# neuromodulation/py_neuromodulation

Measured on AMD Instinct MI355X. Metric: windows/sec (all features), 256 ch @ 1 kHz, higher is better.
Workload: dtype f32; 1 GPU; 256ch/GPU @1kHz, W=1000, hop=100, 1024 hops/step, all 9 hot-path features, 4 bands, notch50+CAR, z-score normalisation; channels_per_gpu=256, features_per_window=9984, parallelism=channel-shard x1, no collective

## Files before the change

### py_neuromodulation_amd/csrc/nmx_engine.inc

```

#include <algorithm>
#include <chrono>
#include <cmath>
#include <cstdio>
#include <cstdlib>
#include <cstring>
#include <map>
#include <string>
#include <thread>
#include <deque>
#include <functional>
#include <mutex>
#include <condition_variable>
#include <pthread.h>
#include <vector>

#include "../../include/nmx.h"
#include "nmx_k_coh.h"
#include "nmx_k_proj.h"

static thread_local std::string g_nmx_err;
static int nmx_fail(int code, const std::string& msg) {
  g_nmx_err = msg;
  return code;
// ... 88 lines not shown
  bool have_sharp = false;
  NmxCohArgs coh{};
  bool have_coh = false;
  float* d_R = nullptr;
  bool car = false;
  float car_diag = 0.f, car_off = 0.f;
  bool rs_ok = false;
  NmxRerefStructArgs rst{};
  int nt_timeosc = 64, nt_bank = 256, nt_thr = 256;
  int chunk_windows = 1024;
  bool sharp_dense_first = false;
  bool thr_wave = true;
  bool thr_fill = true;
  bool fill_split = true;
  bool thr_list_lds = true;
  bool tiny_inline = true;
  bool starts_mod4 = false;
  long long burst_windows_seen = 0;
  Buf thr_slots;
  Buf to_todo;
  Buf rn_qt, rn_qn;
  Buf tap;
  Buf x_in, x_in2[2], x_ref, x_rs, x_rn, rn_mean, rn_scale, x_pf[2], y_notch, yb, out, starts, mask;
  Buf win_pin;
  Buf env[2], swy[2], thr[2], sw_todo[2];
  Buf sw_slab;
  float* d_top = nullptr;
  long long* d_counts = nullptr;
  size_t top_bytes = 0, counts_bytes = 0;
  NmxKalmanArgs kal{};
  bool have_kalman = false;
  NmxResampleArgs rs{};
  bool have_resample = false;
  NmxRawNormArgs rn{};
  bool have_rawnorm = false;
  bool rn_sorted_valid = false;
  long long rn_hops = 0;
  size_t rn_ring_bytes = 0, rn_cnt_bytes = 0, rn_len_bytes = 0;
  std::vector<std::vector<double>> pre_taps;
  int w_in = 0;
  int nt_resample = 256;
  double* d_kf = nullptr;
  size_t kf_bytes = 0;
  be_timer_t timers[9];
// ... 62 lines not shown
```

### py_neuromodulation_amd/csrc/nmx_engine_abi.inc

```

extern "C" {

int nmx_abi_version(void) { return NMX_ABI_VERSION; }
int nmx_device_count(void) { return be_device_count(); }
const char* nmx_last_error(void) { return g_nmx_err.c_str(); }

int nmx_plan_destroy(nmx_plan* plan) {
  Plan* P = (Plan*)plan;
  if (!P) return 0;
  be_set_device(P->device);
  be_sync(P->stream);
  be_sync(P->stream_b);
  be_sync(P->stream_d);
  be_sync(P->stream_f);
  for (void* t : P->tables) be_free(t);
  for (Buf* b : {&P->tap, &P->rn_qt, &P->rn_qn, &P->thr_slots, &P->to_todo, &P->x_dc, &P->x_in, &P->x_ref, &P->x_rs, &P->x_rn, &P->rn_mean, &P->rn_scale, &P->x_pf[0], &P->x_pf[1], &P->sw_todo[0], &P->sw_todo[1], &P->sw_slab, &P->y_notch, &P->env[0], &P->env[1], &P->swy[0], &P->swy[1], &P->yb, &P->thr[0], &P->thr[1], &P->out, &P->starts, &P->mask})
    if (b->p) be_free(b->p);
  if (P->d_top) be_free(P->d_top);
  if (P->d_counts) be_free(P->d_counts);
  if (P->d_R) be_free(P->d_R);
  if (P->d_dc_sub) be_free(P->d_dc_sub);
  if (P->d_dc_pref) be_free(P->d_dc_pref);
  if (P->d_dc_nanv) be_free(P->d_dc_nanv);
  if (P->d_kf) be_free(P->d_kf);
  if (P->rn.ring) be_free(P->rn.ring);
  if (P->rn.count) be_free(P->rn.count);
  if (P->rn.len) be_free(P->rn.len);
  if (P->win_pin.p) be_host_free(P->win_pin.p);
  for (auto& t : P->timers) be_timer_destroy(t);
  be_event_destroy(P->ev_fork);
  be_event_destroy(P->ev_join[0]);
  be_event_destroy(P->ev_join[1]);
  be_event_destroy(P->ev_main[0]);
  be_event_destroy(P->ev_main[1]);
// ... 211 lines not shown
int nmx_state_reset(nmx_plan* plan) {
  Plan* P = (Plan*)plan;
  if (!P) return nmx_fail(NMX_E_INVALID, "null plan");
  dc_reset(*P);
  if (!P->have_bursts && !P->have_kalman && !P->have_rawnorm) return 0;
  be_set_device(P->device);
  be_sync(P->stream);
  if (P->last_stream && P->last_stream != P->stream) be_sync(P->last_stream);
  be_sync(P->stream_b);
  be_sync(P->stream_d);
  be_sync(P->stream_f);
  if (P->have_rawnorm) rawnorm_reset(*P);
  if (P->have_bursts) {
    be_memset_sync(P->d_top, 0, P->top_bytes);
    be_memset_sync(P->d_counts, 0, P->counts_bytes);
    P->burst_windows_seen = 0;
  }
  if (P->have_kalman) kalman_reset(*P);
  return 0;
}

int nmx_state_size(const nmx_plan* plan, int64_t* n_bytes) {
  const Plan* P = (const Plan*)plan;
  if (!P || !n_bytes) return nmx_fail(NMX_E_INVALID, "null argument");
  *n_bytes = (int64_t)(P->top_bytes + P->counts_bytes + P->kf_bytes + dc_state_bytes(*P) + rn_state_bytes(*P));
  return 0;
}

int nmx_state_export(nmx_plan* plan, void* dst, int64_t n_bytes) {
  Plan* P = (Plan*)plan;
// ... 31 lines not shown
  if (P->have_rawnorm && (size_t)n_bytes >= fixed + 2 * sizeof(long long))
    memcpy(&src_cap, (const char*)src + fixed + sizeof(long long), sizeof(long long));
  NMX_REQUIRE(!P->have_rawnorm || (src_cap > 0 && src_cap < (1ll << 31)), "state blob: bad raw-normaliser header");
  NMX_REQUIRE((size_t)n_bytes == fixed + (P->have_rawnorm ? rn_state_bytes_cap(*P, src_cap) : 0), "state size mismatch");
  if (!n_bytes) return 0;
  dc_state_import(*P, (const char*)src + P->top_bytes + P->counts_bytes + P->kf_bytes);
  be_set_device(P->device);
  be_sync(P->stream);
  if (P->last_stream && P->last_stream != P->stream) be_sync(P->last_stream);
  be_sync(P->stream_b);
  be_sync(P->stream_f);
  if (P->have_bursts) {
    be_h2d_sync(P->d_top, src, P->top_bytes);
    be_h2d_sync(P->d_counts, (const char*)src + P->top_bytes, P->counts_bytes);
    memcpy(&P->burst_windows_seen, (const char*)src + P->top_bytes + sizeof(long long), sizeof(long long));
  }
  if (P->have_kalman) be_h2d_sync(P->d_kf, (const char*)src + P->top_bytes + P->counts_bytes, P->kf_bytes);
  if (P->have_rawnorm) {
    const char* q = (const char*)src + P->top_bytes + P->counts_bytes + P->kf_bytes;
    memcpy(&P->rn_hops, q, sizeof(long long)); q += 2 * sizeof(long long);
    const int C = P->d.n_channels, cap = P->rn.cap;
    const float* ring_src = (const float*)q;
    const char* cnt_src = q + (size_t)C * (size_t)src_cap * sizeof(float);
    const char* len_src = cnt_src + P->rn_cnt_bytes;
    if (src_cap == cap) {
      be_h2d_sync(P->rn.ring, ring_src, P->rn_ring_bytes);
    } else {
      std::vector<float> ring((size_t)C * cap, 0.f);
      for (int c = 0; c < C; ++c) {
        long long cnt;
// ... 16 lines not shown
```

### py_neuromodulation_amd/csrc/nmx_engine_plan_state.inc

```
static void rawnorm_reset(Plan& P) {
  be_memset_sync(P.rn.ring, 0, P.rn_ring_bytes);
  be_memset_sync(P.rn.count, 0, P.rn_cnt_bytes);
  be_memset_sync(P.rn.len, 0, P.rn_len_bytes);
  P.rn_hops = 0;
  P.rn_sorted_valid = false;
}

int build_rawnorm(Plan& P) {
  const nmx_plan_desc& d = P.d;
  if (d.raw_norm_method <= 0) return 0;
  NMX_REQUIRE(d.raw_norm_method >= NMX_RAWNORM_MEAN && d.raw_norm_method <= NMX_RAWNORM_POWER,
              "raw normalisation method outside 1..8 (mean, zscore, median, zscore-median, robust, minmax, quantile, power)");
  NMX_REQUIRE(d.raw_norm_n >= 2 && d.raw_norm_add >= 1 && d.raw_norm_add <= d.window,
              "raw normalisation: need N >= 2 and 1 <= int(sfreq / feat_hz) <= window");
  NmxRawNormArgs& A = P.rn;
  A.n_channels = d.n_channels; A.W = d.window;
  A.add = d.raw_norm_add; A.keep = d.raw_norm_n - 1;
  A.cap = std::max(d.window, A.keep) + A.add + 64;
  A.method = d.raw_norm_method; A.clip = d.raw_norm_clip;
  P.rn_ring_bytes = (size_t)d.n_channels * A.cap * sizeof(float);
  P.rn_cnt_bytes = (size_t)d.n_channels * sizeof(long long);
  P.rn_len_bytes = (size_t)d.n_channels * sizeof(int);
  A.ring = (float*)be_alloc(P.rn_ring_bytes);
  A.count = (long long*)be_alloc(P.rn_cnt_bytes);
// ... 66 lines not shown
    A.pad_mode = 0;
    A.n_sw_filters = 1;
    const int L = d.n_pre_taps[i];
    NMX_REQUIRE(L & 1, "pre-filter taps must have odd length");
    const int half = (L - 1) / 2, uh = std::min(half, A.W - 1);
    NmxFilterDev& F = A.f[0];
    F.half = uh;
    F.bp_seglen = 0;
    F.burst_index = -1;
    F.sw_index = 0;
    F.store_raw = 0;
    int rc = build_fir_stage(P, {P.pre_taps[i].data() + (half - uh)}, FirRules{uh, 1024, false, false, 1}, &P.pre[i]);
    if (rc) return rc;
  }
  return 0;
}

int build_bursts(Plan& P) {
  const nmx_plan_desc& d = P.d;
  if (!(d.features & NMX_F_BURSTS)) return 0;
  NMX_REQUIRE(d.n_burst_bands > 0, "bursts enabled without burst bands");
  int nb = 0;
  for (int i = 0; i < d.n_filters; ++i) nb += d.filters[i].burst_index >= 0;
  NMX_REQUIRE(nb == d.n_burst_bands, "every burst band needs exactly one filter");
  NmxBurstThrArgs& T = P.bthr;
  T.n_channels = d.n_channels;
  T.n_bands = d.n_burst_bands;
  T.W = d.window;
  T.q = d.burst_threshold / 100.0;
  NMX_REQUIRE(T.q >= 0.0 && T.q <= 1.0, "burst threshold must be a percentile in [0, 100]");
// ... 28 lines not shown
  S.n_channels = d.n_channels;
  S.n_bands = d.n_burst_bands;
  S.W = d.window;
  S.sfreq = (float)d.sfreq;
  S.seg_s = (float)seg_s;
  S.out_mask = d.burst_out_mask;
  S.cols = cv(d.burst_cols);
  S.off_e = 0;
  S.off_red = al4(d.window + d.window / 16 + 1);
  S.lds_floats = S.off_red + 64;
  const size_t n_state = (size_t)d.n_channels * d.n_burst_bands;
  P.top_bytes = n_state * T.K * sizeof(float);
  P.counts_bytes = n_state * 2 * sizeof(long long);
  P.d_top = (float*)be_alloc(P.top_bytes);
  P.d_counts = (long long*)be_alloc(P.counts_bytes);
  if (!P.d_top || !P.d_counts) return nmx_fail(NMX_E_NOMEM, "burst state allocation failed");
  be_memset_sync(P.d_top, 0, P.top_bytes);
  be_memset_sync(P.d_counts, 0, P.counts_bytes);
  P.have_bursts = true;
  return 0;
}

int build_resample(Plan& P) {
  const nmx_plan_desc& d = P.d;
  if (d.raw_window <= 0) return 0;
  NMX_REQUIRE(d.resample_ratio > 0 && d.resample_ratio != 1.0, "resample_ratio must be positive and != 1");
  NMX_REQUIRE(d.raw_window >= 4 && d.raw_window <= 65336, "raw_window must be in [4, 65 336] samples");
  const double ratio = d.resample_ratio;
  const int W = d.raw_window;
  const int final_len = (int)std::nearbyint(ratio * W);
  NMX_REQUIRE(final_len == d.window, "window must equal round(resample_ratio * raw_window)");
  const int min_add = std::min(W / 8, 100) * 2;
  int n_pad = 1;
// ... 260 lines not shown
```

### py_neuromodulation_amd/csrc/nmx_engine_run.inc

```
static int run_prep_stages(Plan& P, const float*& src, long long& ch_stride, long long& win_stride,
                           const long long*& starts, int nw, int& clean, be_stream_t s, const NmxBankArgs* fuse_bank = nullptr) {
  const int C = P.d.n_channels, W = P.d.window, Wi = P.w_in;
  int rc;
  auto take = [&](const void* y, int w) {
    src = (const float*)y;
    ch_stride = w; win_stride = (long long)C * w; starts = nullptr; clean = 0;
  };
  for (size_t i = 0; i < P.pre.size(); ++i) {
    Buf& dst = P.x_pf[i & 1];
    if ((rc = ensure(dst, (size_t)nw * C * Wi * sizeof(float)))) return rc;
    NmxBankArgs A = P.pre[i].a;
    A.x = src; A.ch_stride = ch_stride; A.win_stride = win_stride; A.starts = starts; A.clean_on_load = clean;
    A.out = nullptr; A.sw_out = (float*)dst.p;
    launch_fir_stage(P, P.pre[i], A, nw * C, s);
    take(dst.p, Wi);
  }
  if (P.have_notch) {
    if ((rc = ensure(P.y_notch, (size_t)nw * C * Wi * sizeof(float)))) return rc;
    NmxBankArgs A = P.notch.a;
    A.x = src; A.ch_stride = ch_stride; A.win_stride = win_stride; A.starts = starts; A.clean_on_load = clean;
    A.out = nullptr; A.y_out = (float*)P.y_notch.p;
#ifndef NMX_HOST_EMU
    if (fuse_bank) launch_notch_bank_fused(P, A, *fuse_bank, nw * C, s);
    else
// ... 19 lines not shown
static int run_chunk(Plan& P, const float* d_x, long long ldx, long long lo, long long hi,
                     const long long* d_starts, int nw, float* d_out, be_stream_t s, bool timed,
                     float* d_pre = nullptr, const int64_t* h_starts = nullptr) {
  const long long n_range = hi - lo;
  const nmx_plan_desc& d = P.d;
  const int C = d.n_channels, W = d.window;
  int rc;
  const int par = (int)(P.chunk_seq & 1);
  if (P.chunk_seq >= 2) {
    be_stream_wait(s, P.ev_join[par]);
    be_stream_wait(s, P.ev_join_d[par]);
  }
  if (P.overlap == 1 && P.chunk_seq >= 1)
    be_stream_wait(s, P.ev_join[par ^ 1]);
  Buf& B_env = P.env[par];
  Buf& B_swy = P.swy[par];
  Buf& B_thr = P.thr[par];
  Buf& B_todo = P.sw_todo[par];
  const float* src = d_x;
  long long ch_stride = ldx, win_stride = 0;
  const long long* starts = d_starts;
  int clean = 1;
  bool raw_live = true;
  const bool tev = timed && nw >= 8;
  if (timed) be_stage_reset();
  if (tev) be_timer_start(P.timers[1], s);
  be_stage(1);
  if (P.d_R) {
    if ((rc = ensure(P.x_ref, (size_t)C * n_range * sizeof(float)))) return rc;
    launch_reref(P, d_x + lo, ldx, (float*)P.x_ref.p, n_range, n_range, s);
// ... 111 lines not shown
    be_event_record(P.ev_fork_d, s);
    be_stream_wait(P.stream_d, P.ev_fork_d);
    if ((rc = launch_sharp(P.stream_d))) return rc;
    be_event_record(P.ev_join_d[par], P.stream_d);
  }
  be_stream_t sb = s;
  be_stage(4);
  if (P.have_bursts) {
    if ((rc = ensure(B_thr, (size_t)nw * C * d.n_burst_bands * sizeof(float)))) return rc;
    if (P.overlap == 1) {
      sb = P.stream_b;
      be_event_record(P.ev_fork, s);
      be_stream_wait(sb, P.ev_fork);
    }
    if (tev) be_timer_start(P.timers[4], sb);
    if (P.bank.w64 || P.bank.a.partitioned) {
      NmxHilbertArgs H = P.hil;
      H.y = (const float*)P.yb.p; H.env = (float*)B_env.p;
      be_launch_hilbert(H, P.hil_kind, (long long)nw * C * d.n_burst_bands, (size_t)H.lds_floats * 4, sb);
    }
    if (P.overlap >= 2) {
      sb = P.stream_b;
      be_event_record(P.ev_fork, s);
      be_stream_wait(sb, P.ev_fork);
    }
    NmxBurstThrArgs T = P.bthr;
    T.env = (const float*)B_env.p; T.thr = (float*)B_thr.p; T.top = P.d_top; T.counts = P.d_counts;
    T.n_windows = nw;
    const int n_seq = C * d.n_burst_bands;
    auto hops = [&](int first, int n) {
      NmxBurstThrArgs X = T;
      X.env = T.env + (size_t)first * n_seq * W;
      X.thr = T.thr + (size_t)first * n_seq;
      X.n_windows = n;
      return X;
    };
    int done = 0;
    if (P.thr_fill && P.burst_windows_seen == 0 && nw >= 2) {
      int n = nmx_burst_fill_hops(T, nw);
#ifndef NMX_HOST_EMU
      if (P.thr_wave)
        for (int k = 1; k < n; ++k)
// ... 17 lines not shown
        for (int k = 1; k < rem; ++k)
          if (nmx_burst_thr_wave_ok(T, seen + k)) { k_fill = k; break; }
      }
#endif
      if (k_fill > 0 && k_fill < rem) {
        be_launch_burst_thr(hops(done, k_fill), n_seq, P.nt_thr, (size_t)T.lds_floats * 4, sb, -1, P.thr_list_lds);
        be_launch_burst_thr(hops(done + k_fill, rem - k_fill), n_seq, P.nt_thr, (size_t)T.lds_floats * 4, sb, seen + k_fill,
                            P.thr_list_lds);
      } else {
        be_launch_burst_thr(hops(done, rem), n_seq, P.nt_thr, (size_t)T.lds_floats * 4, sb, P.thr_wave ? seen : -1, P.thr_list_lds);
      }
    }
    P.burst_windows_seen += nw;
    NmxBurstStatArgs S = P.bstat;
    S.env = (const float*)B_env.p; S.thr = (const float*)B_thr.p; S.out = d_out; S.n_windows = nw;
    be_launch_burst_stat(S, nw * C * d.n_burst_bands, (size_t)S.lds_floats * 4, sb);
    if (tev) be_timer_stop(P.timers[4], sb);
    if (P.overlap) be_event_record(P.ev_join[par], sb);
  }
  if (P.have_to) {
    NmxTimeOscArgs A = P.to;
    A.x = src; A.ch_stride = ch_stride; A.win_stride = win_stride; A.starts = starts;
    A.out = d_out; A.clean_on_load = clean;
    A.starts_mod4 = (!starts || P.starts_mod4) ? 1 : 0;
    A.dcf = dcf;
    if (dcf && !P.to_takes_dc) {
      if ((rc = with_dc())) return rc;
      A.x = src_dc; A.ch_stride = W; A.win_stride = (long long)C * W; A.starts = nullptr; A.clean_on_load = 0; A.dcf = nullptr;
    }
    A.todo = nullptr;
// ... 462 lines not shown
    be_launch_rs64_elem(A, NMX_RS64_MUL, nullptr, cur, L, C, s);
    fft(cur, oth, ld, L, +1, C);
  }
  be_launch_rs64_elem(A, NMX_RS64_OUT, cur, nullptr, final_len, C, s);
  be_d2h_2d_async(y, (size_t)ldy * sizeof(double), d + nx, (size_t)final_len * sizeof(double), (size_t)final_len * sizeof(double),
                  (size_t)C, s);
  rc = be_sync(s);
  be_stream_destroy(s);
  be_free(d);
  return rc ? rc : be_check_launch();
}

int nmx_last_kernels(nmx_plan* plan, int which, char* buf, int64_t n) {
  Plan* P = (Plan*)plan;
  if (!P || !buf || n < 1 || which < 1 || which > 8) return nmx_fail(NMX_E_INVALID, "bad argument");
  const std::string& k = P->kernels[which];
  const size_t m = std::min<size_t>(k.size(), (size_t)n - 1);
  memcpy(buf, k.data(), m);
  buf[m] = 0;
  return 0;
}
```

### py_neuromodulation_amd/csrc/nmx_k_bank_w64.h

```cpp
#pragma once

#include "nmx_k_bank.h"
#include "nmx_k_fft500.h"
#include "nmx_k_sharpwave.h"

#ifdef NMX_HOST_EMU
#define NMX_UNROLL
#else
#define NMX_UNROLL _Pragma("unroll")
#endif

#ifdef NMX_HOST_EMU
#define NMX_SCHED_FENCE() ((void)0)
#else
#define NMX_SCHED_FENCE() __builtin_amdgcn_sched_barrier(0)
#endif

#if defined(NMX_BANK_PROFILE) && !defined(NMX_HOST_EMU)
#define NMX_PROF_DECL long long pf_t = clock64(), pf_acc[8] = {0, 0, 0, 0, 0, 0, 0, 0};
#define NMX_PROF(i) { const long long t_ = clock64(); pf_acc[i] += t_ - pf_t; pf_t = t_; }
#define NMX_PROF_PRINT(w, c)                                                                                          \
  if ((w) == 5 && ((c) == 3 || (c) == 40) && (threadIdx.x & 63) == 0)                                                  \
    printf("bank profile w=%d c=%d: load+fwd %lld | spectral+passA %lld | passB load+dft %lld | passB store %lld | "  \
           "passC %lld | variance %lld | series stores %lld | partners %lld (cycles, whole item, %d filters)\n", (w), (c), pf_acc[0],   \
// ... 643 lines not shown
    NMX_PROF(7)
  }
  NMX_PROF_PRINT(w, c)
}

struct NmxHilbertArgs {
  const float* y;
  float* env;
  int W;
  NmxFft hil_r;
  NmxFft hil_c;
  int hil_full;
  int off_a, off_b, off_y, lds_floats;
  const float* w500_tab;
  const float* w1000_tab;
};

NMX_DEV void nmx_hilbert_item(const NmxHilbertArgs& A, long long item, float* smem) {
  float2* bufA = (float2*)(smem + A.off_a);
  float2* bufB = (float2*)(smem + A.off_b);
  const int W = A.W, Wh = W >> 1;
  const float* src = A.y + item * W;
  float* dst = A.env + item * W;
  if (!A.hil_full) {
    float* ys = smem + A.off_y;
    float* pk = (float*)bufB;
    nmx_stage_row(src, W, [=](int i, float v) { pk[i] = v; ys[i] = v; });
    NMX_SYNC();
    const float2* Zy = nmx_fft_auto<-1, true>(A.hil_r, bufB, bufA, bufB);
    float2* Yb = (Zy == bufA) ? bufB : bufA;
// ... 22 lines not shown
  const float invW = 1.f / (float)W;
  for (int k = NMX_TID; k < W; k += NMX_NT) {
    float2 val = make_float2(0.f, 0.f);
    if (k == 0) val = Zy[0];
    else if (k <= (W - 1) / 2) val = make_float2(2.f * Zy[k].x, 2.f * Zy[k].y);
    Ab[k] = make_float2(val.x * invW, val.y * invW);
  }
  NMX_SYNC();
  float2* Zbuf = (Ab == bufA) ? bufB : bufA;
  const float2* an = nmx_fft_auto<+1, true>(A.hil_c, Ab, Zbuf, Ab);
  for (int i = NMX_TID; i < W; i += NMX_NT) dst[i] = nmx_sqrt_fast(an[i].x * an[i].x + an[i].y * an[i].y);
}

#ifndef NMX_HOST_EMU
#define NMX_W500_LDS_FLOATS (1008 + 1000)
NMX_DEV void nmx_hilbert_w500_item(const NmxHilbertArgs& A, long long item, float* smem) {
  const int l = NMX_TID;
  nmx_c2* hb = (nmx_c2*)smem;
  nmx_c2* ha = hb + 504;
#ifdef NMX_DEBUG_HILBERT_SAMEROW
  const nmx_rsrc rin = nmx_make_rsrc(A.y + (item & 1023) * 1000, 4000);
#else
  const nmx_rsrc rin = nmx_make_rsrc(A.y + item * 1000, 4000);
#endif
  const nmx_rsrc rout = nmx_make_rsrc(A.env + item * 1000, 4000);
  NmxW500TwReg T;
  T.load(A.w500_tab, l);
  nmx_c2 y[8];
#pragma unroll
  for (int q = 0; q < 8; ++q) y[q] = __builtin_amdgcn_raw_buffer_load_b64(rin, 8 * l + 512 * q, 0, 0);
#pragma unroll
  for (int q = 0; q < 8; ++q)
    if (q < 7 || l < 52) hb[l + 64 * q] = y[q];
  NMX_WAVE_FENCE();
  const nmx_c2* ht = nmx_w500_hilbert(ha, hb, T, (const nmx_c2*)A.w500_tab + NMX_W500_TW_N, l);
#pragma unroll
  for (int q = 0; q < 8; ++q) {
    const nmx_c2 h = ht[l + 64 * q];
    const nmx_c2 e = nmx_mk2(nmx_sqrt_fast(y[q].x * y[q].x + h.x * h.x), nmx_sqrt_fast(y[q].y * y[q].y + h.y * h.y));
    __builtin_amdgcn_raw_buffer_store_b64(e, rout, 8 * l + 512 * q, 0, 0);
  }
}
#define NMX_W1000_LDS_FLOATS 2000
NMX_DEV void nmx_hilbert_w1000_item(const NmxHilbertArgs& A, long long item, float* smem) {
  const int l = NMX_TID;
  nmx_c2* hb = (nmx_c2*)smem;
  nmx_c2* ha = hb;
  const nmx_rsrc rin = nmx_make_rsrc(A.y + item * 2000, 8000);
  const nmx_rsrc rout = nmx_make_rsrc(A.env + item * 2000, 8000);
  NmxW1000TwReg T;
  T.load(A.w1000_tab, l);
  nmx_c2 y[16];
#pragma unroll
  for (int q = 0; q < 16; ++q) y[q] = __builtin_amdgcn_raw_buffer_load_b64(rin, 8 * l + 512 * q, 0, 0);
#pragma unroll
  for (int q = 0; q < 16; ++q)
    if (q < 15 || l < 40) hb[l + 64 * q] = y[q];
  NMX_WAVE_FENCE();
  const nmx_c2* ht = nmx_w1000_hilbert(ha, hb, T, (const nmx_c2*)A.w1000_tab + NMX_W1000_TW_N, l);
#pragma unroll
  for (int q = 0; q < 16; ++q) {
    if (!(q < 15 || l < 40)) continue;
    const nmx_c2 h = ht[l + 64 * q];
    const nmx_c2 e = nmx_mk2(nmx_sqrt_fast(y[q].x * y[q].x + h.x * h.x), nmx_sqrt_fast(y[q].y * y[q].y + h.y * h.y));
    __builtin_amdgcn_raw_buffer_store_b64(e, rout, 8 * l + 512 * q, 0, 0);
  }
}
#endif
```

### py_neuromodulation_amd/csrc/nmx_k_burst_stat_reg.h

```cpp
#pragma once

#include "nmx_k_bank_w64.h"
#include "nmx_k_bursts.h"

#ifndef NMX_HOST_EMU
template <int CH>
NMX_DEV void nmx_burst_stat_item_reg(const NmxBurstStatArgs& A, int w, int c, int bi) {
  const int l = NMX_TID, W = A.W;
  const long long item = ((long long)w * A.n_channels + c) * A.n_bands + bi;
  const nmx_rsrc rs = nmx_make_rsrc(A.env + item * W, 4 * W);
  float v[CH];
#pragma unroll
  for (int q = 0; q < CH / 4; ++q) {
    typedef unsigned u4 __attribute__((ext_vector_type(4)));
    const u4 t = __builtin_amdgcn_raw_buffer_load_b128(rs, 4 * (l * CH + 4 * q), 0, 0);
    v[4 * q] = __uint_as_float(t.x); v[4 * q + 1] = __uint_as_float(t.y);
    v[4 * q + 2] = __uint_as_float(t.z); v[4 * q + 3] = __uint_as_float(t.w);
  }
  const float thr = A.thr[item];
  const int i0 = l * CH;
  const int n = W - i0 < 0 ? 0 : (W - i0 > CH ? CH : W - i0);
  float tail = 0.f;
  int zpos = -1;
#pragma unroll
// ... 70 lines not shown
```

### py_neuromodulation_amd/csrc/nmx_k_bursts.h

```cpp
#pragma once

#include "nmx_device.h"
#ifdef NMX_HOST_EMU
#include <cstdio>
#include <cstdlib>
#include <vector>
#endif

struct NmxBurstThrArgs {
  const float* env;
  float* thr;
  float* top;
  long long* counts;
  int n_windows, n_channels, n_bands, W;
  int K;
  int n_ring;
  int overlap;
  double q;
  int P2;
  int off_l0, off_l1, off_p, off_red, lds_floats;
  int list_in_global;
};

NMX_DEV void nmx_bitonic_desc(float* p, int n2) {
  for (int k = 2; k <= n2; k <<= 1) {
    for (int j = k >> 1; j > 0; j >>= 1) {
      for (int i = NMX_TID; i < n2; i += NMX_NT) {
        const int ixj = i ^ j;
        if (ixj > i) {
          const float a = p[i], b = p[ixj];
          const bool desc = ((i & k) == 0);
          if (desc ? (a < b) : (a > b)) {
            p[i] = b;
            p[ixj] = a;
          }
        }
      }
// ... 242 lines not shown
      Lm = nmx_merge_into<CH>(L, Lm, K, ps, ins, nP, vals);
      for (int j = NMX_TID; j < nF; j += NMX_NT) L[Lm + j] = F[nF - 1 - j];
      NMX_SYNC();
      nF = NMX_THR_FREFILL;
      Lm = K - nF;
      nP = 0;
      for (int j = NMX_TID; j < nF; j += NMX_NT) F[j] = L[K - 1 - j];
      NMX_SYNC();
    }
  }
  NMX_SYNC();
  if (!A.list_in_global) for (int i = NMX_TID; i < len; i += NMX_NT) gtop[i] = L[i];
  if (NMX_TID == 0) {
    A.counts[2 * sidx] = total;
    A.counts[2 * sidx + 1] = nwin;
  }
}

#ifndef NMX_HOST_EMU
#define NMX_THRW_PF 16
#define NMX_THRW_I 256
#define NMX_THRW_PF_LL 8
#define NMX_THRW_PF_OF(NR, LL) ((NR) == 2 ? ((LL) ? NMX_THRW_PF_LL : NMX_THRW_PF) : 4)
#define NMX_THRW_LDS_FLOATS_OF(NR, LL) (2 * 256 * (NR) + 3 * ((NR) == 2 ? NMX_THR_P : 512) + NMX_THRW_I + NMX_THRW_PF_OF(NR, LL) * 64 * (NR))
#define NMX_THRW_LDS_FLOATS_NR(NR) NMX_THRW_LDS_FLOATS_OF(NR, false)
#define NMX_THRW_LDS_FLOATS NMX_THRW_LDS_FLOATS_NR(2)

NMX_DEV int nmx_count_ge_lds(const float* l, int n, float v) {
  int lo = 0, hi = n;
  while (lo < hi) {
// ... 360 lines not shown
      }
    }
  }
#ifdef NMX_THRW_PROFILE
  if (lane == 0 && (sidx == 0 || sidx == 311))
    printf("[thrw %lld] hops %d inserts %d flushes %d | cycles: top %lld classify %lld fringe %lld store %lld sort %lld stream %lld recut %lld\n",
           sidx, A.n_windows, n_ins, n_flush, tp[0], tp[1], tp[2], tp[3], tp[4], tp[5], tp[6]);
#endif
  if (LL) {
    NMX_WAVE_FENCE();
    for (int j = lane; j < K; j += 64) Lg[j] = L[j];
  }
  if (lane == 0) {
    A.counts[2 * sidx] = total;
    A.counts[2 * sidx + 1] = nwin;
  }
}
#endif

struct NmxBurstStatArgs {
  const float* env;
  const float* thr;
  float* out;
  int n_outputs, n_windows, n_channels, n_bands, W;
  float sfreq, seg_s;
  unsigned out_mask;
  NmxCols cols;
  int off_e, off_red, lds_floats;
};

#ifdef NMX_HOST_EMU
NMX_DEV double nmx_wave_excl_sum_d(double v, double* total) { *total = v; return 0.0; }
NMX_DEV void nmx_wave_excl_latest(int& pos, double& val) { pos = -1; val = 0.0; }
#else
NMX_DEV double nmx_dpp_d(double v, double ident, int ctrl_sel) {
  const long long vb = __builtin_bit_cast(long long, v), ib = __builtin_bit_cast(long long, ident);
  int lo = (int)(vb & 0xffffffffll), hi = (int)(vb >> 32);
  const int ilo = (int)(ib & 0xffffffffll), ihi = (int)(ib >> 32);
  switch (ctrl_sel) {
    case 0: lo = __builtin_amdgcn_update_dpp(ilo, lo, 0x111, 0xf, 0xf, false); hi = __builtin_amdgcn_update_dpp(ihi, hi, 0x111, 0xf, 0xf, false); break;
    case 1: lo = __builtin_amdgcn_update_dpp(ilo, lo, 0x112, 0xf, 0xf, false); hi = __builtin_amdgcn_update_dpp(ihi, hi, 0x112, 0xf, 0xf, false); break;
    case 2: lo = __builtin_amdgcn_update_dpp(ilo, lo, 0x114, 0xf, 0xf, false); hi = __builtin_amdgcn_update_dpp(ihi, hi, 0x114, 0xf, 0xf, false); break;
    case 3: lo = __builtin_amdgcn_update_dpp(ilo, lo, 0x118, 0xf, 0xf, false); hi = __builtin_amdgcn_update_dpp(ihi, hi, 0x118, 0xf, 0xf, false); break;
    case 4: lo = __builtin_amdgcn_update_dpp(ilo, lo, 0x142, 0xa, 0xf, false); hi = __builtin_amdgcn_update_dpp(ihi, hi, 0x142, 0xa, 0xf, false); break;
// ... 31 lines not shown
    const double tv = nmx_dpp_d(v, 0.0, st);
    if (tp > p) { p = tp; v = tv; }
  }
  pos = nmx_dpp_i(p, -1, 6);
  val = nmx_dpp_d(v, 0.0, 6);
}
#endif

#define NMX_EP(i) ((i) + ((i) >> 4))

NMX_DEV void nmx_burst_stat_item(const NmxBurstStatArgs& A, int w, int c, int bi, float* smem) {
  float* e = smem + A.off_e;
  float* red = smem + A.off_red;
  const int W = A.W;
  const long long item = ((long long)w * A.n_channels + c) * A.n_bands + bi;
  const float* src = A.env + item * W;
  nmx_stage_row(src, W, [=](int i, float v) { e[NMX_EP(i)] = v; });
  NMX_SYNC();
  const float thr = A.thr[item];
  const int chunk = (W + NMX_NT - 1) / NMX_NT;
  const int i0 = NMX_TID * chunk, i1 = (i0 + chunk) < W ? (i0 + chunk) : W;
  double csum = 0.0;
  int zpos = -1;
  double zpre = 0.0;
  for (int i = i0; i < i1; ++i) {
    const float ev = e[NMX_EP(i)];
    csum += (double)ev;
    if (!(ev >= thr)) { zpos = i; zpre = csum; }
  }
  double total;
// ... 61 lines not shown
```

### py_neuromodulation_amd/csrc/nmx_wave.hip

```cpp
#ifndef NMX_NT_FIXED
#error "compile with -DNMX_NT_FIXED=64"
#endif
#include <hip/hip_runtime.h>
#include <cstdio>
#include <cstdlib>

#include <cstdlib>

#include "nmx_k_bursts.h"
#include "nmx_k_bank_w64.h"
#include "nmx_k_burst_stat_reg.h"
#include "nmx_k_scan.h"
#include "nmx_k_td.h"
#include "nmx_k_timeosc_w1000.h"
#include "nmx_k_timeosc_w510.h"
#include "nmx_k_sharpwave.h"

extern __shared__ __attribute__((aligned(16))) float nmx_smem_wave[];

static int waves_per_wg(size_t lds_one, int dflt = 1) {
  const char* v = getenv("NMX_WAVES_PER_WG");
  const int k = (v && atoi(v) >= 1 && atoi(v) <= 4) ? atoi(v) : 0;
  int kk = k ? k : dflt;
  while (kk > 1 && lds_one * kk > 64 * 1024) --kk;
// ... 1 lines not shown
}
#define NMX_WAVE_ITEM(item, smem, n_items, slice)                                                   \
  const int wave_ = __builtin_amdgcn_readfirstlane((int)(threadIdx.x >> 6));                        \
  const int item = (int)blockIdx.x * (int)(blockDim.x >> 6) + wave_;                                \
  if (item >= (n_items)) return;                                                                    \
  float* smem = nmx_smem_wave + wave_ * (slice)

__global__ void __launch_bounds__(256) nmx_kern_burst_stat(const NmxBurstStatArgs A, int n_items, int slice) {
  const int wave = __builtin_amdgcn_readfirstlane((int)(threadIdx.x >> 6));
  const int item = blockIdx.x * (blockDim.x >> 6) + wave;
  if (item >= n_items) return;
  const int bi = item % A.n_bands, r = item / A.n_bands;
  nmx_burst_stat_item(A, r / A.n_channels, r % A.n_channels, bi, nmx_smem_wave + wave * slice);
}

template <int CH>
__global__ void __launch_bounds__(256) nmx_kern_burst_stat_reg(const NmxBurstStatArgs A, int n_items) {
  const int wave = __builtin_amdgcn_readfirstlane((int)(threadIdx.x >> 6));
  const int item = blockIdx.x * 4 + wave;
  if (item >= n_items) return;
  const int bi = item % A.n_bands, r = item / A.n_bands;
  nmx_burst_stat_item_reg<CH>(A, r / A.n_channels, r % A.n_channels, bi);
}

__global__ void __launch_bounds__(256) nmx_kern_sharp(const NmxSharpArgs A, int n_items, int slice) {
  const int wave = __builtin_amdgcn_readfirstlane((int)(threadIdx.x >> 6));
  const int item = blockIdx.x * (blockDim.x >> 6) + wave;
  if (item >= n_items) return;
  const int fi = item % A.n_filters, r = item / A.n_filters;
  nmx_sharp_item(A, r / A.n_channels, r % A.n_channels, fi, nmx_smem_wave + wave * slice);
}

template <int NR, bool LL>
__global__ void __launch_bounds__(64) nmx_kern_burst_thr_wave(const NmxBurstThrArgs A) {
  __builtin_amdgcn_s_setprio(3);
  const int item = blockIdx.x;
  nmx_burst_thr_wave_item<NR, LL>(A, item / A.n_bands, item % A.n_bands, nmx_smem_wave);
// ... 12 lines not shown
  const long long per_round = 256LL * (long long)((160 * 1024) / with_list);
  const bool ll = lds_list && nr == 2 && with_list <= 80 * 1024 && windows_seen < 4096 && (long long)n_items <= 2 * per_round;
  const size_t lds = ll ? with_list : base;
  if (nr == 2) {
    if (ll) hipLaunchKernelGGL((nmx_kern_burst_thr_wave<2, true>), dim3(n_items), dim3(64), lds, s, *A);
    else hipLaunchKernelGGL((nmx_kern_burst_thr_wave<2, false>), dim3(n_items), dim3(64), lds, s, *A);
    nmxi_note_kernel(ll ? "nmx_kern_burst_thr_wave<2, true>" : "nmx_kern_burst_thr_wave<2, false>");
  } else {
    hipLaunchKernelGGL((nmx_kern_burst_thr_wave<4, false>), dim3(n_items), dim3(64), lds, s, *A);
    nmxi_note_kernel("nmx_kern_burst_thr_wave<4, false>");
  }
}

__global__ void __launch_bounds__(256) nmx_kern_hilbert_w500(const NmxHilbertArgs A, int n_items) {
  NMX_WAVE_ITEM(item, smem, n_items, NMX_W500_LDS_FLOATS);
  nmx_hilbert_w500_item(A, (long long)item, smem);
}

extern "C" void nmx_wave_launch_hilbert_w500(const NmxHilbertArgs* A, long long n_items, hipStream_t s) {
  const int k = waves_per_wg((size_t)NMX_W500_LDS_FLOATS * 4);
  hipLaunchKernelGGL(nmx_kern_hilbert_w500, dim3((unsigned)((n_items + k - 1) / k)), dim3(64 * k),
                     (size_t)NMX_W500_LDS_FLOATS * 4 * k, s, *A, (int)n_items);
  nmxi_note_kernel("nmx_kern_hilbert_w500");
}

__global__ void __launch_bounds__(256) nmx_kern_hilbert_w1000(const NmxHilbertArgs A, long long n_items) {
  const int wave = __builtin_amdgcn_readfirstlane((int)(threadIdx.x >> 6));
  const long long item = (long long)blockIdx.x * 4 + wave;
  if (item >= n_items) return;
  nmx_hilbert_w1000_item(A, item, nmx_smem_wave + wave * NMX_W1000_LDS_FLOATS);
}

extern "C" void nmx_wave_launch_hilbert_w1000(const NmxHilbertArgs* A, long long n_items, hipStream_t s) {
  static unsigned long long seen = 0;
  if (nmx_first_on_device(seen))
    (void)hipFuncSetAttribute((const void*)nmx_kern_hilbert_w1000, hipFuncAttributeMaxDynamicSharedMemorySize, 160 * 1024);
  hipLaunchKernelGGL(nmx_kern_hilbert_w1000, dim3((unsigned)((n_items + 3) / 4)), dim3(256), (size_t)4 * NMX_W1000_LDS_FLOATS * 4, s, *A, n_items);
  nmxi_note_kernel("nmx_kern_hilbert_w1000");
}

template <int NB, unsigned SPEC = 0>
__global__ void __launch_bounds__(256) nmx_kern_timeosc_w1000(const NmxTimeOscArgs A, int n_items, int slice) {
  NMX_WAVE_ITEM(item, smem, n_items, slice);
  const int w = nmx_uniform_i(item / A.n_channels), c = nmx_uniform_i(item % A.n_channels);
  NmxW500TwReg T;
  T.load(A.w500_tab, (int)(threadIdx.x & 63));
  NmxTdRegs R;
  nmx_td_load<1000>(A, w, c, R);
  nmx_timeosc_w1000_body<NB, false, NmxW500TwReg, false, SPEC>(A, w, c, R, T, smem);
}

// ... 224 lines not shown
    (void)hipFuncSetAttribute((const void*)nmx_kern_sharp_todo, hipFuncAttributeMaxDynamicSharedMemorySize, 160 * 1024);
  }
  const int blocks = (n_items + 63) / 64;
  const int grid = blocks < 256 * 14 ? blocks : 256 * 14;
  hipLaunchKernelGGL(nmx_kern_sharp_todo, dim3(grid), dim3(64), lds, s, *A, n_items, todo);
  nmxi_note_kernel("nmx_kern_sharp_todo");
}

extern "C" void nmx_wave_launch_burst_stat(const NmxBurstStatArgs* A, int n_items, size_t lds, hipStream_t s) {
  static unsigned long long seen = 0;
  if (nmx_first_on_device(seen)) {
    (void)hipFuncSetAttribute((const void*)nmx_kern_burst_stat, hipFuncAttributeMaxDynamicSharedMemorySize, 160 * 1024);
  }
  if ((A->W & 3) == 0 && A->W <= 2048) {
    if (A->W <= 1024) {
      hipLaunchKernelGGL(nmx_kern_burst_stat_reg<16>, dim3((n_items + 3) / 4), dim3(256), 0, s, *A, n_items);
      nmxi_note_kernel("nmx_kern_burst_stat_reg<16>");
    } else {
      hipLaunchKernelGGL(nmx_kern_burst_stat_reg<32>, dim3((n_items + 3) / 4), dim3(256), 0, s, *A, n_items);
      nmxi_note_kernel("nmx_kern_burst_stat_reg<32>");
    }
    return;
  }
  const int k = waves_per_wg(lds);
  const int slice = (int)((lds / 4 + 3) & ~(size_t)3);
  hipLaunchKernelGGL(nmx_kern_burst_stat, dim3((n_items + k - 1) / k), dim3(64 * k), (size_t)slice * 4 * k, s, *A,
                     n_items, slice);
  nmxi_note_kernel("nmx_kern_burst_stat");
}

extern "C" void nmx_wave_launch_sharp(const NmxSharpArgs* A, int n_items, size_t lds, hipStream_t s) {
  if (A->slab_mode) { nmx_wave_launch_sharp_slab(A, n_items, nullptr, s); return; }
  static unsigned long long seen = 0;
  if (nmx_first_on_device(seen)) {
    (void)hipFuncSetAttribute((const void*)nmx_kern_sharp, hipFuncAttributeMaxDynamicSharedMemorySize, 160 * 1024);
// ... 8 lines not shown
```

Measured before the change: 152,400 windows/s.

## Skip envelope stores and burst stats for rows below running burst threshold floor

```diff
diff --git a/py_neuromodulation_amd/csrc/nmx_engine.inc b/py_neuromodulation_amd/csrc/nmx_engine.inc
--- a/py_neuromodulation_amd/csrc/nmx_engine.inc
+++ b/py_neuromodulation_amd/csrc/nmx_engine.inc
@@ -126,6 +126,9 @@
   bool thr_fill = true;
   bool fill_split = true;
   bool thr_list_lds = true;
+  bool env_sparse = true;
+  bool env_sparse_count = false;
+  long long env_tail_rows = 0, env_rows = 0;
   bool tiny_inline = true;
   bool starts_mod4 = false;
   long long burst_windows_seen = 0;
@@ -136,10 +139,12 @@
   Buf x_in, x_in2[2], x_ref, x_rs, x_rn, rn_mean, rn_scale, x_pf[2], y_notch, yb, out, starts, mask;
   Buf win_pin;
   Buf env[2], swy[2], thr[2], sw_todo[2];
+  Buf env_full[2];
   Buf sw_slab;
   float* d_top = nullptr;
   long long* d_counts = nullptr;
   size_t top_bytes = 0, counts_bytes = 0;
+  float* d_floor = nullptr;
   NmxKalmanArgs kal{};
   bool have_kalman = false;
   NmxResampleArgs rs{};
diff --git a/py_neuromodulation_amd/csrc/nmx_engine_abi.inc b/py_neuromodulation_amd/csrc/nmx_engine_abi.inc
--- a/py_neuromodulation_amd/csrc/nmx_engine_abi.inc
+++ b/py_neuromodulation_amd/csrc/nmx_engine_abi.inc
@@ -14,10 +14,11 @@
   be_sync(P->stream_d);
   be_sync(P->stream_f);
   for (void* t : P->tables) be_free(t);
-  for (Buf* b : {&P->tap, &P->rn_qt, &P->rn_qn, &P->thr_slots, &P->to_todo, &P->x_dc, &P->x_in, &P->x_ref, &P->x_rs, &P->x_rn, &P->rn_mean, &P->rn_scale, &P->x_pf[0], &P->x_pf[1], &P->sw_todo[0], &P->sw_todo[1], &P->sw_slab, &P->y_notch, &P->env[0], &P->env[1], &P->swy[0], &P->swy[1], &P->yb, &P->thr[0], &P->thr[1], &P->out, &P->starts, &P->mask})
+  for (Buf* b : {&P->tap, &P->rn_qt, &P->rn_qn, &P->thr_slots, &P->to_todo, &P->x_dc, &P->x_in, &P->x_ref, &P->x_rs, &P->x_rn, &P->rn_mean, &P->rn_scale, &P->x_pf[0], &P->x_pf[1], &P->sw_todo[0], &P->sw_todo[1], &P->sw_slab, &P->y_notch, &P->env[0], &P->env[1], &P->env_full[0], &P->env_full[1], &P->swy[0], &P->swy[1], &P->yb, &P->thr[0], &P->thr[1], &P->out, &P->starts, &P->mask})
     if (b->p) be_free(b->p);
   if (P->d_top) be_free(P->d_top);
   if (P->d_counts) be_free(P->d_counts);
+  if (P->d_floor) be_free(P->d_floor);
   if (P->d_R) be_free(P->d_R);
   if (P->d_dc_sub) be_free(P->d_dc_sub);
   if (P->d_dc_pref) be_free(P->d_dc_pref);
@@ -259,6 +260,7 @@
   if (P->have_bursts) {
     be_memset_sync(P->d_top, 0, P->top_bytes);
     be_memset_sync(P->d_counts, 0, P->counts_bytes);
+    burst_floor_reset(*P);
     P->burst_windows_seen = 0;
   }
   if (P->have_kalman) kalman_reset(*P);
@@ -320,6 +322,7 @@
     be_h2d_sync(P->d_top, src, P->top_bytes);
     be_h2d_sync(P->d_counts, (const char*)src + P->top_bytes, P->counts_bytes);
     memcpy(&P->burst_windows_seen, (const char*)src + P->top_bytes + sizeof(long long), sizeof(long long));
+    burst_floor_reset(*P);
   }
   if (P->have_kalman) be_h2d_sync(P->d_kf, (const char*)src + P->top_bytes + P->counts_bytes, P->kf_bytes);
   if (P->have_rawnorm) {
diff --git a/py_neuromodulation_amd/csrc/nmx_engine_plan_state.inc b/py_neuromodulation_amd/csrc/nmx_engine_plan_state.inc
--- a/py_neuromodulation_amd/csrc/nmx_engine_plan_state.inc
+++ b/py_neuromodulation_amd/csrc/nmx_engine_plan_state.inc
@@ -104,6 +104,11 @@
     if (rc) return rc;
   }
   return 0;
+}
+
+void burst_floor_reset(Plan& P) {
+  const std::vector<float> f((size_t)P.d.n_channels * P.d.n_burst_bands, -INFINITY);
+  be_h2d_sync(P.d_floor, f.data(), f.size() * sizeof(float));
 }
 
 int build_bursts(Plan& P) {
@@ -162,9 +167,17 @@
   P.counts_bytes = n_state * 2 * sizeof(long long);
   P.d_top = (float*)be_alloc(P.top_bytes);
   P.d_counts = (long long*)be_alloc(P.counts_bytes);
-  if (!P.d_top || !P.d_counts) return nmx_fail(NMX_E_NOMEM, "burst state allocation failed");
+  P.d_floor = (float*)be_alloc(n_state * sizeof(float));
+  if (!P.d_top || !P.d_counts || !P.d_floor) return nmx_fail(NMX_E_NOMEM, "burst state allocation failed");
   be_memset_sync(P.d_top, 0, P.top_bytes);
   be_memset_sync(P.d_counts, 0, P.counts_bytes);
+  burst_floor_reset(P);
+#ifdef NMX_HOST_EMU
+  P.env_sparse = false;
+#else
+  P.env_sparse = env_int("NMX_BURST_ENV_SPARSE", 1) != 0;
+  P.env_sparse_count = env_int("NMX_BURST_ENV_SPARSE", 1) == 2;
+#endif
   P.have_bursts = true;
   return 0;
 }
diff --git a/py_neuromodulation_amd/csrc/nmx_engine_run.inc b/py_neuromodulation_amd/csrc/nmx_engine_run.inc
--- a/py_neuromodulation_amd/csrc/nmx_engine_run.inc
+++ b/py_neuromodulation_amd/csrc/nmx_engine_run.inc
@@ -57,6 +57,7 @@
   if (P.overlap == 1 && P.chunk_seq >= 1)
     be_stream_wait(s, P.ev_join[par ^ 1]);
   Buf& B_env = P.env[par];
+  Buf& B_full = P.env_full[par];
   Buf& B_swy = P.swy[par];
   Buf& B_thr = P.thr[par];
   Buf& B_todo = P.sw_todo[par];
@@ -198,10 +199,24 @@
       be_stream_wait(sb, P.ev_fork);
     }
     if (tev) be_timer_start(P.timers[4], sb);
+    const unsigned char* env_full = nullptr;
     if (P.bank.w64 || P.bank.a.partitioned) {
       NmxHilbertArgs H = P.hil;
       H.y = (const float*)P.yb.p; H.env = (float*)B_env.p;
+      if (P.env_sparse && (P.hil_kind == NMX_HIL_W500 || P.hil_kind == NMX_HIL_W1000)) {
+        if ((rc = ensure(B_full, (size_t)nw * C * d.n_burst_bands))) return rc;
+        H.floor = P.d_floor; H.full = (unsigned char*)B_full.p;
+        H.n_seq = C * d.n_burst_bands; H.overlap = P.bthr.overlap;
+        env_full = H.full;
+      }
       be_launch_hilbert(H, P.hil_kind, (long long)nw * C * d.n_burst_bands, (size_t)H.lds_floats * 4, sb);
+      if (env_full && P.env_sparse_count) {
+        std::vector<unsigned char> f((size_t)nw * C * d.n_burst_bands);
+        if ((rc = be_sync(sb))) return rc;
+        be_d2h_sync(f.data(), env_full, f.size());
+        for (unsigned char v : f) P.env_tail_rows += v == 0;
+        P.env_rows += (long long)f.size();
+      }
     }
     if (P.overlap >= 2) {
       sb = P.stream_b;
@@ -210,6 +225,7 @@
     }
     NmxBurstThrArgs T = P.bthr;
     T.env = (const float*)B_env.p; T.thr = (float*)B_thr.p; T.top = P.d_top; T.counts = P.d_counts;
+    T.floor = P.d_floor;
     T.n_windows = nw;
     const int n_seq = C * d.n_burst_bands;
     auto hops = [&](int first, int n) {
@@ -257,6 +273,7 @@
     P.burst_windows_seen += nw;
     NmxBurstStatArgs S = P.bstat;
     S.env = (const float*)B_env.p; S.thr = (const float*)B_thr.p; S.out = d_out; S.n_windows = nw;
+    S.full = env_full;
     be_launch_burst_stat(S, nw * C * d.n_burst_bands, (size_t)S.lds_floats * 4, sb);
     if (tev) be_timer_stop(P.timers[4], sb);
     if (P.overlap) be_event_record(P.ev_join[par], sb);
@@ -749,7 +766,9 @@
 int nmx_last_kernels(nmx_plan* plan, int which, char* buf, int64_t n) {
   Plan* P = (Plan*)plan;
   if (!P || !buf || n < 1 || which < 1 || which > 8) return nmx_fail(NMX_E_INVALID, "bad argument");
-  const std::string& k = P->kernels[which];
+  std::string k = P->kernels[which];
+  if (which == 4 && P->env_sparse_count)
+    k += (k.empty() ? "" : ",") + std::string("env_tail_rows=") + std::to_string(P->env_tail_rows) + "/" + std::to_string(P->env_rows);
   const size_t m = std::min<size_t>(k.size(), (size_t)n - 1);
   memcpy(buf, k.data(), m);
   buf[m] = 0;
diff --git a/py_neuromodulation_amd/csrc/nmx_k_bank_w64.h b/py_neuromodulation_amd/csrc/nmx_k_bank_w64.h
--- a/py_neuromodulation_amd/csrc/nmx_k_bank_w64.h
+++ b/py_neuromodulation_amd/csrc/nmx_k_bank_w64.h
@@ -681,6 +681,9 @@
   int off_a, off_b, off_y, lds_floats;
   const float* w500_tab;
   const float* w1000_tab;
+  const float* floor;
+  unsigned char* full;
+  int n_seq, overlap;
 };
 
 NMX_DEV void nmx_hilbert_item(const NmxHilbertArgs& A, long long item, float* smem) {
@@ -733,6 +736,7 @@
 
 #ifndef NMX_HOST_EMU
 #define NMX_W500_LDS_FLOATS (1008 + 1000)
+template <bool SPARSE>
 NMX_DEV void nmx_hilbert_w500_item(const NmxHilbertArgs& A, long long item, float* smem) {
   const int l = NMX_TID;
   nmx_c2* hb = (nmx_c2*)smem;
@@ -743,6 +747,7 @@
   const nmx_rsrc rin = nmx_make_rsrc(A.y + item * 1000, 4000);
 #endif
   const nmx_rsrc rout = nmx_make_rsrc(A.env + item * 1000, 4000);
+  const float fl = SPARSE ? A.floor[(int)item % A.n_seq] : 0.f;
   NmxW500TwReg T;
   T.load(A.w500_tab, l);
   nmx_c2 y[8];
@@ -753,6 +758,22 @@
     if (q < 7 || l < 52) hb[l + 64 * q] = y[q];
   NMX_WAVE_FENCE();
   const nmx_c2* ht = nmx_w500_hilbert(ha, hb, T, (const nmx_c2*)A.w500_tab + NMX_W500_TW_N, l);
+  if (SPARSE) {
+    bool hit = !(fl > -INFINITY);
+#pragma unroll
+    for (int q = 0; q < 8; ++q) {
+      const nmx_c2 h = ht[l + 64 * q];
+      y[q] = nmx_mk2(nmx_sqrt_fast(y[q].x * y[q].x + h.x * h.x), nmx_sqrt_fast(y[q].y * y[q].y + h.y * h.y));
+      hit = hit || ((q < 7 || l < 52) && (y[q].x >= fl || y[q].y >= fl));
+    }
+    const bool row = __ballot(hit) != 0ull;
+    const int keep = 1000 - A.overlap;
+#pragma unroll
+    for (int q = 0; q < 8; ++q)
+      if (row || 2 * (l + 64 * q) + 2 > keep) __builtin_amdgcn_raw_buffer_store_b64(y[q], rout, 8 * l + 512 * q, 0, 0);
+    if (l == 0) A.full[item] = row ? 1 : 0;
+    return;
+  }
 #pragma unroll
   for (int q = 0; q < 8; ++q) {
     const nmx_c2 h = ht[l + 64 * q];
@@ -761,12 +782,14 @@
   }
 }
 #define NMX_W1000_LDS_FLOATS 2000
+template <bool SPARSE>
 NMX_DEV void nmx_hilbert_w1000_item(const NmxHilbertArgs& A, long long item, float* smem) {
   const int l = NMX_TID;
   nmx_c2* hb = (nmx_c2*)smem;
   nmx_c2* ha = hb;
   const nmx_rsrc rin = nmx_make_rsrc(A.y + item * 2000, 8000);
   const nmx_rsrc rout = nmx_make_rsrc(A.env + item * 2000, 8000);
+  const float fl = SPARSE ? A.floor[(int)(item % (long long)A.n_seq)] : 0.f;
   NmxW1000TwReg T;
   T.load(A.w1000_tab, l);
   nmx_c2 y[16];
@@ -777,6 +800,24 @@
     if (q < 15 || l < 40) hb[l + 64 * q] = y[q];
   NMX_WAVE_FENCE();
   const nmx_c2* ht = nmx_w1000_hilbert(ha, hb, T, (const nmx_c2*)A.w1000_tab + NMX_W1000_TW_N, l);
+  if (SPARSE) {
+    bool hit = !(fl > -INFINITY);
+#pragma unroll
+    for (int q = 0; q < 16; ++q) {
+      if (!(q < 15 || l < 40)) continue;
+      const nmx_c2 h = ht[l + 64 * q];
+      y[q] = nmx_mk2(nmx_sqrt_fast(y[q].x * y[q].x + h.x * h.x), nmx_sqrt_fast(y[q].y * y[q].y + h.y * h.y));
+      hit = hit || y[q].x >= fl || y[q].y >= fl;
+    }
+    const bool row = __ballot(hit) != 0ull;
+    const int keep = 2000 - A.overlap;
+#pragma unroll
+    for (int q = 0; q < 16; ++q)
+      if ((q < 15 || l < 40) && (row || 2 * (l + 64 * q) + 2 > keep))
+        __builtin_amdgcn_raw_buffer_store_b64(y[q], rout, 8 * l + 512 * q, 0, 0);
+    if (l == 0) A.full[item] = row ? 1 : 0;
+    return;
+  }
 #pragma unroll
   for (int q = 0; q < 16; ++q) {
     if (!(q < 15 || l < 40)) continue;
diff --git a/py_neuromodulation_amd/csrc/nmx_k_burst_stat_reg.h b/py_neuromodulation_amd/csrc/nmx_k_burst_stat_reg.h
--- a/py_neuromodulation_amd/csrc/nmx_k_burst_stat_reg.h
+++ b/py_neuromodulation_amd/csrc/nmx_k_burst_stat_reg.h
@@ -4,10 +4,14 @@
 #include "nmx_k_bursts.h"
 
 #ifndef NMX_HOST_EMU
-template <int CH>
+template <int CH, bool SPARSE = false>
 NMX_DEV void nmx_burst_stat_item_reg(const NmxBurstStatArgs& A, int w, int c, int bi) {
   const int l = NMX_TID, W = A.W;
   const long long item = ((long long)w * A.n_channels + c) * A.n_bands + bi;
+  if (SPARSE && !__builtin_amdgcn_readfirstlane((int)A.full[item])) {
+    if (l == 0) nmx_burst_stat_zero(A, w, c, bi);
+    return;
+  }
   const nmx_rsrc rs = nmx_make_rsrc(A.env + item * W, 4 * W);
   float v[CH];
 #pragma unroll
diff --git a/py_neuromodulation_amd/csrc/nmx_k_bursts.h b/py_neuromodulation_amd/csrc/nmx_k_bursts.h
--- a/py_neuromodulation_amd/csrc/nmx_k_bursts.h
+++ b/py_neuromodulation_amd/csrc/nmx_k_bursts.h
@@ -20,7 +20,10 @@
   int P2;
   int off_l0, off_l1, off_p, off_red, lds_floats;
   int list_in_global;
+  float* floor;
 };
+
+NMX_DEV float nmx_burst_floor_of(float v) { return (v - v == 0.f) ? v : -INFINITY; }
 
 NMX_DEV void nmx_bitonic_desc(float* p, int n2) {
   for (int k = 2; k <= n2; k <<= 1) {
@@ -293,6 +296,8 @@
   if (NMX_TID == 0) {
     A.counts[2 * sidx] = total;
     A.counts[2 * sidx + 1] = nwin;
+    if (A.floor && A.n_windows > 0)
+      A.floor[sidx] = (total >= m_ring && ia_ring >= 0 && ia_ring < len) ? nmx_burst_floor_of(L[ia_ring]) : -INFINITY;
   }
 }
 
@@ -683,6 +688,7 @@
   if (lane == 0) {
     A.counts[2 * sidx] = total;
     A.counts[2 * sidx + 1] = nwin;
+    if (A.floor && A.n_windows > 0) A.floor[sidx] = nmx_burst_floor_of(F[fh + ja]);
   }
 }
 #endif
@@ -696,7 +702,18 @@
   unsigned out_mask;
   NmxCols cols;
   int off_e, off_red, lds_floats;
+  const unsigned char* full;
 };
+
+NMX_DEV void nmx_burst_stat_zero(const NmxBurstStatArgs& A, int w, int c, int bi) {
+  float* row = A.out + (long long)w * A.n_outputs;
+  int col = A.cols.base + c * A.cols.ch_stride + bi * A.cols.a_stride;
+  for (int s = 0; s < 6; ++s)
+    if (A.out_mask & (1u << s)) {
+      row[col] = 0.f;
+      col += A.cols.b_stride;
+    }
+}
 
 #ifdef NMX_HOST_EMU
 NMX_DEV double nmx_wave_excl_sum_d(double v, double* total) { *total = v; return 0.0; }
@@ -758,6 +775,10 @@
   float* red = smem + A.off_red;
   const int W = A.W;
   const long long item = ((long long)w * A.n_channels + c) * A.n_bands + bi;
+  if (A.full && !A.full[item]) {
+    if (NMX_TID == 0) nmx_burst_stat_zero(A, w, c, bi);
+    return;
+  }
   const float* src = A.env + item * W;
   nmx_stage_row(src, W, [=](int i, float v) { e[NMX_EP(i)] = v; });
   NMX_SYNC();
diff --git a/py_neuromodulation_amd/csrc/nmx_wave.hip b/py_neuromodulation_amd/csrc/nmx_wave.hip
--- a/py_neuromodulation_amd/csrc/nmx_wave.hip
+++ b/py_neuromodulation_amd/csrc/nmx_wave.hip
@@ -39,13 +39,13 @@
   nmx_burst_stat_item(A, r / A.n_channels, r % A.n_channels, bi, nmx_smem_wave + wave * slice);
 }
 
-template <int CH>
+template <int CH, bool SPARSE = false>
 __global__ void __launch_bounds__(256) nmx_kern_burst_stat_reg(const NmxBurstStatArgs A, int n_items) {
   const int wave = __builtin_amdgcn_readfirstlane((int)(threadIdx.x >> 6));
   const int item = blockIdx.x * 4 + wave;
   if (item >= n_items) return;
   const int bi = item % A.n_bands, r = item / A.n_bands;
-  nmx_burst_stat_item_reg<CH>(A, r / A.n_channels, r % A.n_channels, bi);
+  nmx_burst_stat_item_reg<CH, SPARSE>(A, r / A.n_channels, r % A.n_channels, bi);
 }
 
 __global__ void __launch_bounds__(256) nmx_kern_sharp(const NmxSharpArgs A, int n_items, int slice) {
@@ -88,11 +88,21 @@
 
 __global__ void __launch_bounds__(256) nmx_kern_hilbert_w500(const NmxHilbertArgs A, int n_items) {
   NMX_WAVE_ITEM(item, smem, n_items, NMX_W500_LDS_FLOATS);
-  nmx_hilbert_w500_item(A, (long long)item, smem);
+  nmx_hilbert_w500_item<false>(A, (long long)item, smem);
+}
+__global__ void __launch_bounds__(256) nmx_kern_hilbert_w500_sparse(const NmxHilbertArgs A, int n_items) {
+  NMX_WAVE_ITEM(item, smem, n_items, NMX_W500_LDS_FLOATS);
+  nmx_hilbert_w500_item<true>(A, (long long)item, smem);
 }
 
 extern "C" void nmx_wave_launch_hilbert_w500(const NmxHilbertArgs* A, long long n_items, hipStream_t s) {
   const int k = waves_per_wg((size_t)NMX_W500_LDS_FLOATS * 4);
+  if (A->full) {
+    hipLaunchKernelGGL(nmx_kern_hilbert_w500_sparse, dim3((unsigned)((n_items + k - 1) / k)), dim3(64 * k),
+                       (size_t)NMX_W500_LDS_FLOATS * 4 * k, s, *A, (int)n_items);
+    nmxi_note_kernel("nmx_kern_hilbert_w500_sparse");
+    return;
+  }
   hipLaunchKernelGGL(nmx_kern_hilbert_w500, dim3((unsigned)((n_items + k - 1) / k)), dim3(64 * k),
                      (size_t)NMX_W500_LDS_FLOATS * 4 * k, s, *A, (int)n_items);
   nmxi_note_kernel("nmx_kern_hilbert_w500");
@@ -102,13 +112,26 @@
   const int wave = __builtin_amdgcn_readfirstlane((int)(threadIdx.x >> 6));
   const long long item = (long long)blockIdx.x * 4 + wave;
   if (item >= n_items) return;
-  nmx_hilbert_w1000_item(A, item, nmx_smem_wave + wave * NMX_W1000_LDS_FLOATS);
+  nmx_hilbert_w1000_item<false>(A, item, nmx_smem_wave + wave * NMX_W1000_LDS_FLOATS);
+}
+__global__ void __launch_bounds__(256) nmx_kern_hilbert_w1000_sparse(const NmxHilbertArgs A, long long n_items) {
+  const int wave = __builtin_amdgcn_readfirstlane((int)(threadIdx.x >> 6));
+  const long long item = (long long)blockIdx.x * 4 + wave;
+  if (item >= n_items) return;
+  nmx_hilbert_w1000_item<true>(A, item, nmx_smem_wave + wave * NMX_W1000_LDS_FLOATS);
 }
 
 extern "C" void nmx_wave_launch_hilbert_w1000(const NmxHilbertArgs* A, long long n_items, hipStream_t s) {
   static unsigned long long seen = 0;
-  if (nmx_first_on_device(seen))
+  if (nmx_first_on_device(seen)) {
     (void)hipFuncSetAttribute((const void*)nmx_kern_hilbert_w1000, hipFuncAttributeMaxDynamicSharedMemorySize, 160 * 1024);
+    (void)hipFuncSetAttribute((const void*)nmx_kern_hilbert_w1000_sparse, hipFuncAttributeMaxDynamicSharedMemorySize, 160 * 1024);
+  }
+  if (A->full) {
+    hipLaunchKernelGGL(nmx_kern_hilbert_w1000_sparse, dim3((unsigned)((n_items + 3) / 4)), dim3(256), (size_t)4 * NMX_W1000_LDS_FLOATS * 4, s, *A, n_items);
+    nmxi_note_kernel("nmx_kern_hilbert_w1000_sparse");
+    return;
+  }
   hipLaunchKernelGGL(nmx_kern_hilbert_w1000, dim3((unsigned)((n_items + 3) / 4)), dim3(256), (size_t)4 * NMX_W1000_LDS_FLOATS * 4, s, *A, n_items);
   nmxi_note_kernel("nmx_kern_hilbert_w1000");
 }
@@ -363,11 +386,13 @@
   }
   if ((A->W & 3) == 0 && A->W <= 2048) {
     if (A->W <= 1024) {
-      hipLaunchKernelGGL(nmx_kern_burst_stat_reg<16>, dim3((n_items + 3) / 4), dim3(256), 0, s, *A, n_items);
-      nmxi_note_kernel("nmx_kern_burst_stat_reg<16>");
+      if (A->full) hipLaunchKernelGGL((nmx_kern_burst_stat_reg<16, true>), dim3((n_items + 3) / 4), dim3(256), 0, s, *A, n_items);
+      else hipLaunchKernelGGL(nmx_kern_burst_stat_reg<16>, dim3((n_items + 3) / 4), dim3(256), 0, s, *A, n_items);
+      nmxi_note_kernel(A->full ? "nmx_kern_burst_stat_reg_sparse<16>" : "nmx_kern_burst_stat_reg<16>");
     } else {
-      hipLaunchKernelGGL(nmx_kern_burst_stat_reg<32>, dim3((n_items + 3) / 4), dim3(256), 0, s, *A, n_items);
-      nmxi_note_kernel("nmx_kern_burst_stat_reg<32>");
+      if (A->full) hipLaunchKernelGGL((nmx_kern_burst_stat_reg<32, true>), dim3((n_items + 3) / 4), dim3(256), 0, s, *A, n_items);
+      else hipLaunchKernelGGL(nmx_kern_burst_stat_reg<32>, dim3((n_items + 3) / 4), dim3(256), 0, s, *A, n_items);
+      nmxi_note_kernel(A->full ? "nmx_kern_burst_stat_reg_sparse<32>" : "nmx_kern_burst_stat_reg<32>");
     }
     return;
   }
```

New measurement: 163,600 windows/s (median of 6 runs). 7.4% higher.
